# radiocosmology/driftscan

Hardware: AMD Instinct MI355X
Metric: m-blocks/sec (BT-gen + SVD + KL) (higher is better)
Workload: dtype f64

## Files before the change

driftscan_amd/csrc/dm_chol.hip:

```cpp
#include "dm_common.h"
#include "dm_kernels.h"

#include <algorithm>

namespace {

constexpr int NB = 32;

struct chol_desc {
  cplx* A; int ld; int n;
};

__global__ __launch_bounds__(256) void potf2_kernel(const chol_desc* __restrict__ ds, int k0, int* __restrict__ info) {
  __shared__ cplx T[NB][NB + 1];
  __shared__ cplx Lo[NB][NB + 1];
  const chol_desc d = ds[blockIdx.x];
  if (k0 >= d.n) return;
  if (info[blockIdx.x] != 0) return;
  const int nb = min(NB, d.n - k0);
  const int tid = threadIdx.x;
  for (int idx = tid; idx < NB * NB; idx += 256) {
    int r = idx / NB, c = idx % NB;
    T[r][c] = (r < nb && c < nb && c <= r) ? d.A[(size_t)(k0 + r) * d.ld + k0 + c] : make_double2(0.0, 0.0);
    Lo[r][c] = make_double2(0.0, 0.0);
  }
  int fail = 0;
  for (int j = 0; j < nb; ++j) {
    __syncthreads();
    const double djj = T[j][j].x;
    if (!(djj > 0.0) || !isfinite(djj)) {
      fail = j + 1;
      break;
    }
    const double inv = 1.0 / djj, invs = 1.0 / sqrt(djj);
    if (tid >= j && tid < nb) Lo[tid][j] = tid == j ? make_double2(sqrt(djj), 0.0) : cscale(T[tid][j], invs);
    for (int idx = tid; idx < NB * NB; idx += 256) {
      int r = idx / NB, c = idx % NB;
      if (c > j && c <= r && r < nb) T[r][c] = csub(T[r][c], cscale(cmulc(T[r][j], T[c][j]), inv));
    }
  }
  if (fail) {
    if (tid == 0) info[blockIdx.x] = k0 + fail;
    return;
  }
  __syncthreads();
  for (int idx = tid; idx < NB * NB; idx += 256) {
    int r = idx / NB, c = idx % NB;
    if (r < nb && c < nb) {
      cplx v = (c <= r) ? Lo[r][c] : make_double2(0.0, 0.0);
      if (c == r) v.y = 0.0;
      d.A[(size_t)(k0 + r) * d.ld + k0 + c] = v;
    }
  }
}

__global__ __launch_bounds__(256) void panel_trsm_kernel(const chol_desc* __restrict__ ds, int k0,
                                                         const int* __restrict__ info) {
  __shared__ cplx Lk[NB][NB + 1];
  __shared__ cplx R[64][NB + 1];
  const chol_desc d = ds[blockIdx.y];
  if (k0 + NB >= d.n) return;
  if (info[blockIdx.y] != 0) return;
  const int r0 = k0 + NB + blockIdx.x * 64;
  if (r0 >= d.n) return;
  const int tid = threadIdx.x;
  for (int idx = tid; idx < NB * NB; idx += 256) {
    int r = idx / NB, c = idx % NB;
    Lk[r][c] = d.A[(size_t)(k0 + r) * d.ld + k0 + c];
  }
  for (int idx = tid; idx < 64 * NB; idx += 256) {
    int r = idx / NB, c = idx % NB;
    R[r][c] = (r0 + r < d.n) ? d.A[(size_t)(r0 + r) * d.ld + k0 + c] : make_double2(0.0, 0.0);
  }
  __syncthreads();
  if (tid < 64) {
    const int r = tid;
    cplx x[NB];
#pragma unroll
    for (int c = 0; c < NB; ++c) x[c] = R[r][c];
#pragma unroll
    for (int c = 0; c < NB; ++c) {
      x[c] = cscale(x[c], 1.0 / Lk[c][c].x);
#pragma unroll
      for (int j = c + 1; j < NB; ++j) x[j] = csub(x[j], cmulc(x[c], Lk[j][c]));
    }
#pragma unroll
    for (int c = 0; c < NB; ++c) R[r][c] = x[c];
  }
  __syncthreads();
  for (int idx = tid; idx < 64 * NB; idx += 256) {
    int r = idx / NB, c = idx % NB;
    if (r0 + r < d.n) d.A[(size_t)(r0 + r) * d.ld + k0 + c] = R[r][c];
  }
}

__global__ void zero_upper_kernel(const chol_desc* __restrict__ ds) {
  const chol_desc d = ds[blockIdx.z];
  const int r = blockIdx.y, c = blockIdx.x * blockDim.x + threadIdx.x;
  if (r < d.n && c < d.n && c > r) d.A[(size_t)r * d.ld + c] = make_double2(0.0, 0.0);
}

struct trsm_desc {
  const cplx* L; int ldl; int n; cplx* B; int ldb; int nrhs;
};

template <bool CONJTRANS>
__global__ __launch_bounds__(256) void diag_solve_kernel(const trsm_desc* __restrict__ ds, int s, int nblk, int upper_only) {
  __shared__ cplx Lk[NB][NB + 1];
  const trsm_desc d = ds[blockIdx.y];
  int k0;
  if (!CONJTRANS) {
    k0 = s * NB;
  } else {
    const int pn = (d.n + NB - 1) / NB;
    if (s < nblk - pn) return;
    k0 = (pn - 1 - (s - (nblk - pn))) * NB;
  }
  if (k0 >= d.n || k0 < 0) return;
  const int nb = min(NB, d.n - k0);
  const int col = blockIdx.x * 256 + threadIdx.x;
  const int first_col = upper_only ? (k0 / (2 * NB)) * (2 * NB) : 0;
  if ((int)(blockIdx.x + 1) * 256 <= first_col) return;
  for (int idx = threadIdx.x; idx < NB * NB; idx += 256) {
    int r = idx / NB, c = idx % NB;
    Lk[r][c] = (r < nb && c < nb) ? d.L[(size_t)(k0 + r) * d.ldl + k0 + c] : make_double2(0.0, 0.0);
  }
  __syncthreads();
  if (col >= d.nrhs || (col / 64 + 1) * 64 <= first_col) return;
  cplx x[NB];
#pragma unroll
  for (int r = 0; r < NB; ++r) x[r] = (r < nb) ? d.B[(size_t)(k0 + r) * d.ldb + col] : make_double2(0.0, 0.0);
  if (!CONJTRANS) {
#pragma unroll
    for (int r = 0; r < NB; ++r) {
      if (r < nb) {
        x[r] = cscale(x[r], 1.0 / Lk[r][r].x);
#pragma unroll
        for (int j = r + 1; j < NB; ++j) x[j] = csub(x[j], cmul(Lk[j][r], x[r]));
      }
    }
  } else {
#pragma unroll
    for (int rr = 0; rr < NB; ++rr) {
      const int r = NB - 1 - rr;
      if (r < nb) {
        x[r] = cscale(x[r], 1.0 / Lk[r][r].x);
#pragma unroll
        for (int j = 0; j < r; ++j) x[j] = csub(x[j], cmul(cconj(Lk[r][j]), x[r]));
      }
    }
  }
#pragma unroll
  for (int r = 0; r < NB; ++r)
    if (r < nb) d.B[(size_t)(k0 + r) * d.ldb + col] = x[r];
}

}

int dm_potrf_batched(dm_ctx* ctx, const std::vector<dm_mat>& mats, int* info_dev) {
  const int nbatch = (int)mats.size();
  if (nbatch == 0) return DM_OK;
  dm_ws_scope ws_scope__(ctx);
  const size_t mark = ws_scope__.mark;
  std::vector<chol_desc> ds(nbatch);
  int maxn = 0;
  for (int i = 0; i < nbatch; ++i) {
    ds[i] = chol_desc{mats[i].p, mats[i].ld, mats[i].n};
    maxn = std::max(maxn, mats[i].n);
  }
  chol_desc* dd = dm_ws_upload(ctx, ds);
  if (!dd) return DM_ENOMEM;
  DM_HIP(ctx, hipMemsetAsync(info_dev, 0, sizeof(int) * nbatch, ctx->stream));
  dm_gemm_chain chain(ctx);
  for (int pass = 0; pass < 2; ++pass) {
    if (pass == 1) DM_TRY(chain.upload());
    for (int k0 = 0; k0 < maxn; k0 += 2 * NB) {
      for (int half = 0; half < 2; ++half) {
        const int kk = k0 + half * NB;
        if (kk >= maxn) break;
        if (!chain.dry) DM_PLAUNCH(ctx, DM_PROF_CHOL, potf2_kernel, dim3(nbatch), dim3(256), 0, ctx->stream, dd, kk, info_dev);
        if (kk + NB >= maxn) break;
        const int rt = (maxn - kk - NB + 63) / 64;
        if (!chain.dry) DM_PLAUNCH(ctx, DM_PROF_CHOL, panel_trsm_kernel, dim3(rt, nbatch), dim3(256), 0, ctx->stream, dd, kk, info_dev);
        if (half == 0) {
          DM_TRY(chain.gemm([&](std::vector<dm_gemm_desc>& g) {
            for (int i = 0; i < nbatch; ++i) {
              const int rem = mats[i].n - kk - NB;
              if (rem <= 0) continue;
              cplx* L21 = mats[i].p + (size_t)(kk + NB) * mats[i].ld + kk;
              cplx* A22 = mats[i].p + (size_t)(kk + NB) * mats[i].ld + (kk + NB);
              g.push_back(dm_gemm_make(L21, mats[i].ld, 1, false, L21, 1, mats[i].ld, true, A22, mats[i].ld, rem,
                                       std::min(NB, rem), NB, -1.0, 1.0));
            }
          }));
        }
      }
      const int k2 = k0 + 2 * NB;
      if (k2 < maxn) {
        DM_TRY(chain.gemm([&](std::vector<dm_gemm_desc>& g) {
          for (int i = 0; i < nbatch; ++i) {
            const int rem = mats[i].n - k2;
            if (rem <= 0) continue;
            cplx* L21 = mats[i].p + (size_t)k2 * mats[i].ld + k0;
            cplx* A22 = mats[i].p + (size_t)k2 * mats[i].ld + k2;
            g.push_back(dm_gemm_make(L21, mats[i].ld, 1, false, L21, 1, mats[i].ld, true, A22, mats[i].ld, rem, rem,
                                     2 * NB, -1.0, 1.0, nullptr, DM_GEMM_LOWER));
          }
        }));
      }
    }
  }
  DM_PLAUNCH(ctx, DM_PROF_CHOL, zero_upper_kernel, dim3((maxn + 255) / 256, maxn, nbatch), dim3(256), 0, ctx->stream, dd);
  DM_HIP(ctx, hipGetLastError());
  (void)mark;
  return DM_OK;
}

namespace {
int trsm_pass(dm_ctx* ctx, const std::vector<dm_trsm_problem>& probs, bool conjtrans, bool upper_only, dm_gemm_chain& chain,
              const trsm_desc* dd) {
  const int nbatch = (int)probs.size();
  int maxn = 0, maxrhs = 0;
  for (int i = 0; i < nbatch; ++i) {
    maxn = std::max(maxn, probs[i].n);
    maxrhs = std::max(maxrhs, probs[i].nrhs);
  }
  const int ct = (maxrhs + 255) / 256;
  const int NB2 = 2 * NB;
  const int nblk = (maxn + NB2 - 1) / NB2;
  const int nblk32 = (maxn + NB - 1) / NB;
  for (int s = 0; s < nblk; ++s) {
    DM_TRY(chain.gemm([&](std::vector<dm_gemm_desc>& g) {
    for (int i = 0; i < nbatch; ++i) {
      const dm_trsm_problem& P = probs[i];
      const int pn = (P.n + NB2 - 1) / NB2;
      if (!conjtrans) {
        if (s == 0 || s >= pn) continue;
        const int size = s & -s;
        const int r0 = s * NB2, r1 = std::min((s + size) * NB2, P.n);
        const int c0 = (s - size) * NB2;
        const int j0 = upper_only ? std::min(r0, P.nrhs) : 0;
        if (P.nrhs - j0 <= 0) continue;
        g.push_back(dm_gemm_make(P.L + (size_t)r0 * P.ldl + c0, P.ldl, 1, false, P.B + (size_t)c0 * P.ldb + j0, P.ldb, 1,
                                 false, P.B + (size_t)r0 * P.ldb + j0, P.ldb, r1 - r0, P.nrhs - j0, size * NB2, -1.0,
                                 1.0));
      } else {
        if (s < nblk - pn) continue;
        const int u = s - (nblk - pn);
        if (u == 0) continue;
        const int kb = pn - 1 - u;
        const int size = u & -u;
        const int t0 = std::max(kb - size + 1, 0) * NB2, t1 = (kb + 1) * NB2;
        const int k1 = t1, k2 = std::min((kb + 1 + size) * NB2, P.n);
        g.push_back(dm_gemm_make(P.L + (size_t)k1 * P.ldl + t0, 1, P.ldl, true, P.B + (size_t)k1 * P.ldb, P.ldb, 1,
                                 false, P.B + (size_t)t0 * P.ldb, P.ldb, t1 - t0, P.nrhs, k2 - k1, -1.0, 1.0));
      }
    }
    }));
    for (int half = 0; half < 2; ++half) {
      const int h = conjtrans ? 1 - half : half;
      int s32;
      if (!conjtrans) s32 = 2 * s + h;
      else s32 = 2 * s + half;
      if (chain.dry) {
      } else if (!conjtrans)
        DM_PLAUNCH(ctx, DM_PROF_CHOL, diag_solve_kernel<false>, dim3(ct, nbatch), dim3(256), 0, ctx->stream, dd, s32, nblk32,
                           upper_only ? 1 : 0);
      else
        DM_PLAUNCH(ctx, DM_PROF_CHOL, diag_solve_kernel<true>, dim3(ct, nbatch), dim3(256), 0, ctx->stream, dd, s32, 2 * nblk, 0);
      if (half == 0) {
        DM_TRY(chain.gemm([&](std::vector<dm_gemm_desc>& g2) {
        for (int i = 0; i < nbatch; ++i) {
          const dm_trsm_problem& P = probs[i];
          const int pn = (P.n + NB2 - 1) / NB2;
          if (!conjtrans) {
            const int k0 = s * NB2, k1 = k0 + NB;
            if (k1 >= P.n) continue;
            const int nb = std::min(NB, P.n - k1);
            const int j0 = upper_only ? std::min(k0, P.nrhs) : 0;
            if (P.nrhs - j0 <= 0) continue;
            g2.push_back(dm_gemm_make(P.L + (size_t)k1 * P.ldl + k0, P.ldl, 1, false, P.B + (size_t)k0 * P.ldb + j0,
                                      P.ldb, 1, false, P.B + (size_t)k1 * P.ldb + j0, P.ldb, nb, P.nrhs - j0, NB, -1.0,
                                      1.0));
          } else {
            if (s < nblk - pn) continue;
            const int kb = pn - 1 - (s - (nblk - pn));
            const int k0 = kb * NB2, k1 = k0 + NB;
            if (k1 >= P.n) continue;
            const int nb2 = std::min(NB, P.n - k1);
            g2.push_back(dm_gemm_make(P.L + (size_t)k1 * P.ldl + k0, 1, P.ldl, true, P.B + (size_t)k1 * P.ldb, P.ldb,
                                      1, false, P.B + (size_t)k0 * P.ldb, P.ldb, NB, P.nrhs, nb2, -1.0, 1.0));
          }
        }
        }));
      }
    }
  }
  return DM_OK;
}
}

int dm_trsm_plan_build(dm_ctx* ctx, const std::vector<dm_trsm_problem>& probs, bool conjtrans, bool upper_only, dm_trsm_plan& plan) {
  if (conjtrans) upper_only = false;
  plan.probs = probs;
  plan.conjtrans = conjtrans;
  plan.upper_only = upper_only;
  plan.chain.reset(new dm_gemm_chain(ctx));
  plan.empty = true;
  for (const auto& P : probs)
    if (P.n > 0 && P.nrhs > 0) plan.empty = false;
  if (plan.empty) return DM_OK;
  return trsm_pass(ctx, plan.probs, conjtrans, upper_only, *plan.chain, nullptr);
}

int dm_trsm_plan_run(dm_ctx* ctx, dm_trsm_plan& plan) {
  if (plan.empty || !plan.chain) return DM_OK;
  const int nbatch = (int)plan.probs.size();
  std::vector<trsm_desc> ds(nbatch);
  for (int i = 0; i < nbatch; ++i)
    ds[i] = trsm_desc{plan.probs[i].L, plan.probs[i].ldl, plan.probs[i].n, plan.probs[i].B, plan.probs[i].ldb, plan.probs[i].nrhs};
  trsm_desc* dd = dm_ws_upload(ctx, ds);
  if (!dd) return DM_ENOMEM;
  DM_TRY(plan.chain->upload());
  DM_TRY(trsm_pass(ctx, plan.probs, plan.conjtrans, plan.upper_only, *plan.chain, dd));
  DM_HIP(ctx, hipGetLastError());
  return DM_OK;
}

int dm_trsm_left_lower_batched(dm_ctx* ctx, const std::vector<dm_trsm_problem>& probs, bool conjtrans, bool upper_only) {
  dm_trsm_plan plan;
  DM_TRY(dm_trsm_plan_build(ctx, probs, conjtrans, upper_only, plan));
  return dm_trsm_plan_run(ctx, plan);
}
```

Baseline: 1116.

## Use 64-wide diagonal blocks with quad-thread solves in Cholesky and TRSM

Replaces the 32-wide potf2/panel-trsm/diag-solve kernels with 64-wide versions. The diagonal block is stored in packed-triangular shared memory, and each row or column is solved by four cooperating lanes that exchange values with shuffles. This removes the intermediate 32-wide GEMM updates and halves the number of kernel launches per block step. In exchange each diagonal step does more serial work, and the per-thread register arrays and the triangular-index arithmetic add cost.

```diff
diff --git a/driftscan_amd/csrc/dm_chol.hip b/driftscan_amd/csrc/dm_chol.hip
--- a/driftscan_amd/csrc/dm_chol.hip
+++ b/driftscan_amd/csrc/dm_chol.hip
@@ -5,38 +5,39 @@
 
 namespace {
 
-constexpr int NB = 32;
+constexpr int NB2 = 64;
+
+constexpr int TRI64 = NB2 * (NB2 + 1) / 2;
+__device__ __forceinline__ int tri(int r, int c) { return r * (r + 1) / 2 + c; }
 
 struct chol_desc {
   cplx* A; int ld; int n;
 };
 
-__global__ __launch_bounds__(256) void potf2_kernel(const chol_desc* __restrict__ ds, int k0, int* __restrict__ info) {
-  __shared__ cplx T[NB][NB + 1];
-  __shared__ cplx Lo[NB][NB + 1];
+__global__ __launch_bounds__(256) void potf2_64_kernel(const chol_desc* __restrict__ ds, int k0, int* __restrict__ info) {
+  __shared__ cplx T[TRI64];
   const chol_desc d = ds[blockIdx.x];
   if (k0 >= d.n) return;
   if (info[blockIdx.x] != 0) return;
-  const int nb = min(NB, d.n - k0);
+  const int nb = min(NB2, d.n - k0);
   const int tid = threadIdx.x;
-  for (int idx = tid; idx < NB * NB; idx += 256) {
-    int r = idx / NB, c = idx % NB;
-    T[r][c] = (r < nb && c < nb && c <= r) ? d.A[(size_t)(k0 + r) * d.ld + k0 + c] : make_double2(0.0, 0.0);
-    Lo[r][c] = make_double2(0.0, 0.0);
-  }
+  for (int idx = tid; idx < NB2 * NB2; idx += 256) {
+    const int r = idx / NB2, c = idx % NB2;
+    if (c <= r) T[tri(r, c)] = (r < nb) ? d.A[(size_t)(k0 + r) * d.ld + k0 + c] : make_double2(0.0, 0.0);
+  }
+  const int r = tid >> 2, q = tid & 3;
   int fail = 0;
   for (int j = 0; j < nb; ++j) {
     __syncthreads();
-    const double djj = T[j][j].x;
+    const double djj = T[tri(j, j)].x;
     if (!(djj > 0.0) || !isfinite(djj)) {
       fail = j + 1;
       break;
     }
-    const double inv = 1.0 / djj, invs = 1.0 / sqrt(djj);
-    if (tid >= j && tid < nb) Lo[tid][j] = tid == j ? make_double2(sqrt(djj), 0.0) : cscale(T[tid][j], invs);
-    for (int idx = tid; idx < NB * NB; idx += 256) {
-      int r = idx / NB, c = idx % NB;
-      if (c > j && c <= r && r < nb) T[r][c] = csub(T[r][c], cscale(cmulc(T[r][j], T[c][j]), inv));
+    const double inv = 1.0 / djj;
+    if (r > j && r < nb) {
+      const cplx trj = T[tri(r, j)];
+      for (int c = j + 1 + q; c <= r; c += 4) T[tri(r, c)] = csub(T[tri(r, c)], cscale(cmulc(trj, T[tri(c, j)]), inv));
     }
   }
   if (fail) {
@@ -44,54 +45,77 @@
     return;
   }
   __syncthreads();
-  for (int idx = tid; idx < NB * NB; idx += 256) {
-    int r = idx / NB, c = idx % NB;
-    if (r < nb && c < nb) {
-      cplx v = (c <= r) ? Lo[r][c] : make_double2(0.0, 0.0);
-      if (c == r) v.y = 0.0;
-      d.A[(size_t)(k0 + r) * d.ld + k0 + c] = v;
-    }
-  }
-}
-
-__global__ __launch_bounds__(256) void panel_trsm_kernel(const chol_desc* __restrict__ ds, int k0,
-                                                         const int* __restrict__ info) {
-  __shared__ cplx Lk[NB][NB + 1];
-  __shared__ cplx R[64][NB + 1];
+  for (int idx = tid; idx < NB2 * NB2; idx += 256) {
+    const int rr = idx / NB2, c = idx % NB2;
+    if (rr < nb && c < nb) {
+      cplx v = make_double2(0.0, 0.0);
+      if (c == rr) v.x = sqrt(T[tri(c, c)].x);
+      else if (c < rr) v = cscale(T[tri(rr, c)], 1.0 / sqrt(T[tri(c, c)].x));
+      d.A[(size_t)(k0 + rr) * d.ld + k0 + c] = v;
+    }
+  }
+}
+
+template <bool BACK, bool CONJL>
+__device__ __forceinline__ void quad_solve64(const cplx* Lk, const double* rdiag, int nb, int q, cplx (&x)[NB2 / 4]) {
+  constexpr int NQ = NB2 / 4;
+#pragma unroll
+  for (int rr = 0; rr < NB2; ++rr) {
+    const int r = BACK ? NB2 - 1 - rr : rr;
+    if (r < nb) {
+      const int ir = r / 4;
+      const cplx v = cscale(x[ir], rdiag[r]);
+      cplx xr;
+      xr.x = __shfl(v.x, r & 3, 4);
+      xr.y = __shfl(v.y, r & 3, 4);
+      if (q == (r & 3)) x[ir] = xr;
+      if (!BACK) {
+#pragma unroll
+        for (int i = ir; i < NQ; ++i) {
+          const int j = 4 * i + q;
+          if (i > ir || q > (r & 3)) {
+            const cplx l = Lk[tri(j, r)];
+            x[i] = csub(x[i], cmul(CONJL ? cconj(l) : l, xr));
+          }
+        }
+      } else {
+#pragma unroll
+        for (int i = 0; i <= ir; ++i) {
+          const int j = 4 * i + q;
+          if (i < ir || q < (r & 3)) x[i] = csub(x[i], cmul(cconj(Lk[tri(r, j)]), xr));
+        }
+      }
+    }
+  }
+}
+
+__global__ __launch_bounds__(256) void panel_trsm64_kernel(const chol_desc* __restrict__ ds, int k0,
+                                                           const int* __restrict__ info) {
+  __shared__ cplx Lk[TRI64];
   const chol_desc d = ds[blockIdx.y];
-  if (k0 + NB >= d.n) return;
+  if (k0 + NB2 >= d.n) return;
   if (info[blockIdx.y] != 0) return;
-  const int r0 = k0 + NB + blockIdx.x * 64;
+  const int r0 = k0 + NB2 + blockIdx.x * 64;
   if (r0 >= d.n) return;
   const int tid = threadIdx.x;
-  for (int idx = tid; idx < NB * NB; idx += 256) {
-    int r = idx / NB, c = idx % NB;
-    Lk[r][c] = d.A[(size_t)(k0 + r) * d.ld + k0 + c];
-  }
-  for (int idx = tid; idx < 64 * NB; idx += 256) {
-    int r = idx / NB, c = idx % NB;
-    R[r][c] = (r0 + r < d.n) ? d.A[(size_t)(r0 + r) * d.ld + k0 + c] : make_double2(0.0, 0.0);
-  }
+  for (int idx = tid; idx < NB2 * NB2; idx += 256) {
+    const int r = idx / NB2, c = idx % NB2;
+    if (c <= r) Lk[tri(r, c)] = d.A[(size_t)(k0 + r) * d.ld + k0 + c];
+  }
+  __shared__ double rdiag[NB2];
+  if (tid < NB2) rdiag[tid] = 1.0 / d.A[(size_t)(k0 + tid) * d.ld + k0 + tid].x;
   __syncthreads();
-  if (tid < 64) {
-    const int r = tid;
-    cplx x[NB];
-#pragma unroll
-    for (int c = 0; c < NB; ++c) x[c] = R[r][c];
-#pragma unroll
-    for (int c = 0; c < NB; ++c) {
-      x[c] = cscale(x[c], 1.0 / Lk[c][c].x);
-#pragma unroll
-      for (int j = c + 1; j < NB; ++j) x[j] = csub(x[j], cmulc(x[c], Lk[j][c]));
-    }
-#pragma unroll
-    for (int c = 0; c < NB; ++c) R[r][c] = x[c];
-  }
-  __syncthreads();
-  for (int idx = tid; idx < 64 * NB; idx += 256) {
-    int r = idx / NB, c = idx % NB;
-    if (r0 + r < d.n) d.A[(size_t)(r0 + r) * d.ld + k0 + c] = R[r][c];
-  }
+  const int row = r0 + (tid >> 2), q = tid & 3;
+  if (row >= d.n) return;
+  cplx* a = d.A + (size_t)row * d.ld + k0;
+  cplx x[NB2 / 4];
+#pragma unroll
+  for (int i = 0; i < NB2 / 4; ++i) x[i] = a[4 * i + q];
+  int nb = NB2;
+  asm volatile("" : "+s"(nb));
+  quad_solve64<false, true>(Lk, rdiag, nb, q, x);
+#pragma unroll
+  for (int i = 0; i < NB2 / 4; ++i) a[4 * i + q] = x[i];
 }
 
 __global__ void zero_upper_kernel(const chol_desc* __restrict__ ds) {
@@ -105,54 +129,39 @@
 };
 
 template <bool CONJTRANS>
-__global__ __launch_bounds__(256) void diag_solve_kernel(const trsm_desc* __restrict__ ds, int s, int nblk, int upper_only) {
-  __shared__ cplx Lk[NB][NB + 1];
+__global__ __launch_bounds__(256) void diag_solve64_kernel(const trsm_desc* __restrict__ ds, int s, int nblk, int upper_only) {
+  __shared__ cplx Lk[TRI64];
   const trsm_desc d = ds[blockIdx.y];
   int k0;
   if (!CONJTRANS) {
-    k0 = s * NB;
+    k0 = s * NB2;
   } else {
-    const int pn = (d.n + NB - 1) / NB;
+    const int pn = (d.n + NB2 - 1) / NB2;
     if (s < nblk - pn) return;
-    k0 = (pn - 1 - (s - (nblk - pn))) * NB;
+    k0 = (pn - 1 - (s - (nblk - pn))) * NB2;
   }
   if (k0 >= d.n || k0 < 0) return;
-  const int nb = min(NB, d.n - k0);
-  const int col = blockIdx.x * 256 + threadIdx.x;
-  const int first_col = upper_only ? (k0 / (2 * NB)) * (2 * NB) : 0;
-  if ((int)(blockIdx.x + 1) * 256 <= first_col) return;
-  for (int idx = threadIdx.x; idx < NB * NB; idx += 256) {
-    int r = idx / NB, c = idx % NB;
-    Lk[r][c] = (r < nb && c < nb) ? d.L[(size_t)(k0 + r) * d.ldl + k0 + c] : make_double2(0.0, 0.0);
-  }
+  const int nb = min(NB2, d.n - k0);
+  const int col = blockIdx.x * 64 + (threadIdx.x >> 2), q = threadIdx.x & 3;
+  const int first_col = upper_only ? k0 : 0;
+  if ((int)(blockIdx.x + 1) * 64 <= first_col) return;
+  for (int idx = threadIdx.x; idx < NB2 * NB2; idx += 256) {
+    const int r = idx / NB2, c = idx % NB2;
+    if (c <= r) Lk[tri(r, c)] = (r < nb) ? d.L[(size_t)(k0 + r) * d.ldl + k0 + c] : make_double2(0.0, 0.0);
+  }
+  __shared__ double rdiag[NB2];
+  if (threadIdx.x < nb) rdiag[threadIdx.x] = 1.0 / d.L[(size_t)(k0 + threadIdx.x) * d.ldl + k0 + threadIdx.x].x;
   __syncthreads();
-  if (col >= d.nrhs || (col / 64 + 1) * 64 <= first_col) return;
-  cplx x[NB];
-#pragma unroll
-  for (int r = 0; r < NB; ++r) x[r] = (r < nb) ? d.B[(size_t)(k0 + r) * d.ldb + col] : make_double2(0.0, 0.0);
-  if (!CONJTRANS) {
-#pragma unroll
-    for (int r = 0; r < NB; ++r) {
-      if (r < nb) {
-        x[r] = cscale(x[r], 1.0 / Lk[r][r].x);
-#pragma unroll
-        for (int j = r + 1; j < NB; ++j) x[j] = csub(x[j], cmul(Lk[j][r], x[r]));
-      }
-    }
-  } else {
-#pragma unroll
-    for (int rr = 0; rr < NB; ++rr) {
-      const int r = NB - 1 - rr;
-      if (r < nb) {
-        x[r] = cscale(x[r], 1.0 / Lk[r][r].x);
-#pragma unroll
-        for (int j = 0; j < r; ++j) x[j] = csub(x[j], cmul(cconj(Lk[r][j]), x[r]));
-      }
-    }
-  }
-#pragma unroll
-  for (int r = 0; r < NB; ++r)
-    if (r < nb) d.B[(size_t)(k0 + r) * d.ldb + col] = x[r];
+  if (col >= d.nrhs || col < first_col) return;
+  cplx* b = d.B + (size_t)k0 * d.ldb + col;
+  const size_t ldb = d.ldb;
+  cplx x[NB2 / 4];
+#pragma unroll
+  for (int i = 0; i < NB2 / 4; ++i) x[i] = (4 * i + q < nb) ? b[(4 * i + q) * ldb] : make_double2(0.0, 0.0);
+  quad_solve64<CONJTRANS, false>(Lk, rdiag, nb, q, x);
+#pragma unroll
+  for (int i = 0; i < NB2 / 4; ++i)
+    if (4 * i + q < nb) b[(4 * i + q) * ldb] = x[i];
 }
 
 }
@@ -174,40 +183,22 @@
   dm_gemm_chain chain(ctx);
   for (int pass = 0; pass < 2; ++pass) {
     if (pass == 1) DM_TRY(chain.upload());
-    for (int k0 = 0; k0 < maxn; k0 += 2 * NB) {
-      for (int half = 0; half < 2; ++half) {
-        const int kk = k0 + half * NB;
-        if (kk >= maxn) break;
-        if (!chain.dry) DM_PLAUNCH(ctx, DM_PROF_CHOL, potf2_kernel, dim3(nbatch), dim3(256), 0, ctx->stream, dd, kk, info_dev);
-        if (kk + NB >= maxn) break;
-        const int rt = (maxn - kk - NB + 63) / 64;
-        if (!chain.dry) DM_PLAUNCH(ctx, DM_PROF_CHOL, panel_trsm_kernel, dim3(rt, nbatch), dim3(256), 0, ctx->stream, dd, kk, info_dev);
-        if (half == 0) {
-          DM_TRY(chain.gemm([&](std::vector<dm_gemm_desc>& g) {
-            for (int i = 0; i < nbatch; ++i) {
-              const int rem = mats[i].n - kk - NB;
-              if (rem <= 0) continue;
-              cplx* L21 = mats[i].p + (size_t)(kk + NB) * mats[i].ld + kk;
-              cplx* A22 = mats[i].p + (size_t)(kk + NB) * mats[i].ld + (kk + NB);
-              g.push_back(dm_gemm_make(L21, mats[i].ld, 1, false, L21, 1, mats[i].ld, true, A22, mats[i].ld, rem,
-                                       std::min(NB, rem), NB, -1.0, 1.0));
-            }
-          }));
+    for (int k0 = 0; k0 < maxn; k0 += NB2) {
+      if (!chain.dry) DM_PLAUNCH(ctx, DM_PROF_CHOL, potf2_64_kernel, dim3(nbatch), dim3(256), 0, ctx->stream, dd, k0, info_dev);
+      const int k2 = k0 + NB2;
+      if (k2 >= maxn) break;
+      const int rt = (maxn - k2 + 63) / 64;
+      if (!chain.dry) DM_PLAUNCH(ctx, DM_PROF_CHOL, panel_trsm64_kernel, dim3(rt, nbatch), dim3(256), 0, ctx->stream, dd, k0, info_dev);
+      DM_TRY(chain.gemm([&](std::vector<dm_gemm_desc>& g) {
+        for (int i = 0; i < nbatch; ++i) {
+          const int rem = mats[i].n - k2;
+          if (rem <= 0) continue;
+          cplx* L21 = mats[i].p + (size_t)k2 * mats[i].ld + k0;
+          cplx* A22 = mats[i].p + (size_t)k2 * mats[i].ld + k2;
+          g.push_back(dm_gemm_make(L21, mats[i].ld, 1, false, L21, 1, mats[i].ld, true, A22, mats[i].ld, rem, rem, NB2, -1.0,
+                                   1.0, nullptr, DM_GEMM_LOWER));
         }
-      }
-      const int k2 = k0 + 2 * NB;
-      if (k2 < maxn) {
-        DM_TRY(chain.gemm([&](std::vector<dm_gemm_desc>& g) {
-          for (int i = 0; i < nbatch; ++i) {
-            const int rem = mats[i].n - k2;
-            if (rem <= 0) continue;
-            cplx* L21 = mats[i].p + (size_t)k2 * mats[i].ld + k0;
-            cplx* A22 = mats[i].p + (size_t)k2 * mats[i].ld + k2;
-            g.push_back(dm_gemm_make(L21, mats[i].ld, 1, false, L21, 1, mats[i].ld, true, A22, mats[i].ld, rem, rem,
-                                     2 * NB, -1.0, 1.0, nullptr, DM_GEMM_LOWER));
-          }
-        }));
-      }
+      }));
     }
   }
   DM_PLAUNCH(ctx, DM_PROF_CHOL, zero_upper_kernel, dim3((maxn + 255) / 256, maxn, nbatch), dim3(256), 0, ctx->stream, dd);
@@ -225,10 +216,8 @@
     maxn = std::max(maxn, probs[i].n);
     maxrhs = std::max(maxrhs, probs[i].nrhs);
   }
-  const int ct = (maxrhs + 255) / 256;
-  const int NB2 = 2 * NB;
+  const int ct = (maxrhs + 63) / 64;
   const int nblk = (maxn + NB2 - 1) / NB2;
-  const int nblk32 = (maxn + NB - 1) / NB;
   for (int s = 0; s < nblk; ++s) {
     DM_TRY(chain.gemm([&](std::vector<dm_gemm_desc>& g) {
     for (int i = 0; i < nbatch; ++i) {
@@ -257,44 +246,12 @@
       }
     }
     }));
-    for (int half = 0; half < 2; ++half) {
-      const int h = conjtrans ? 1 - half : half;
-      int s32;
-      if (!conjtrans) s32 = 2 * s + h;
-      else s32 = 2 * s + half;
-      if (chain.dry) {
-      } else if (!conjtrans)
-        DM_PLAUNCH(ctx, DM_PROF_CHOL, diag_solve_kernel<false>, dim3(ct, nbatch), dim3(256), 0, ctx->stream, dd, s32, nblk32,
-                           upper_only ? 1 : 0);
-      else
-        DM_PLAUNCH(ctx, DM_PROF_CHOL, diag_solve_kernel<true>, dim3(ct, nbatch), dim3(256), 0, ctx->stream, dd, s32, 2 * nblk, 0);
-      if (half == 0) {
-        DM_TRY(chain.gemm([&](std::vector<dm_gemm_desc>& g2) {
-        for (int i = 0; i < nbatch; ++i) {
-          const dm_trsm_problem& P = probs[i];
-          const int pn = (P.n + NB2 - 1) / NB2;
-          if (!conjtrans) {
-            const int k0 = s * NB2, k1 = k0 + NB;
-            if (k1 >= P.n) continue;
-            const int nb = std::min(NB, P.n - k1);
-            const int j0 = upper_only ? std::min(k0, P.nrhs) : 0;
-            if (P.nrhs - j0 <= 0) continue;
-            g2.push_back(dm_gemm_make(P.L + (size_t)k1 * P.ldl + k0, P.ldl, 1, false, P.B + (size_t)k0 * P.ldb + j0,
-                                      P.ldb, 1, false, P.B + (size_t)k1 * P.ldb + j0, P.ldb, nb, P.nrhs - j0, NB, -1.0,
-                                      1.0));
-          } else {
-            if (s < nblk - pn) continue;
-            const int kb = pn - 1 - (s - (nblk - pn));
-            const int k0 = kb * NB2, k1 = k0 + NB;
-            if (k1 >= P.n) continue;
-            const int nb2 = std::min(NB, P.n - k1);
-            g2.push_back(dm_gemm_make(P.L + (size_t)k1 * P.ldl + k0, 1, P.ldl, true, P.B + (size_t)k1 * P.ldb, P.ldb,
-                                      1, false, P.B + (size_t)k0 * P.ldb, P.ldb, NB, P.nrhs, nb2, -1.0, 1.0));
-          }
-        }
-        }));
-      }
-    }
+    if (chain.dry) {
+    } else if (!conjtrans)
+      DM_PLAUNCH(ctx, DM_PROF_CHOL, diag_solve64_kernel<false>, dim3(ct, nbatch), dim3(256), 0, ctx->stream, dd, s, nblk,
+                 upper_only ? 1 : 0);
+    else
+      DM_PLAUNCH(ctx, DM_PROF_CHOL, diag_solve64_kernel<true>, dim3(ct, nbatch), dim3(256), 0, ctx->stream, dd, s, nblk, 0);
   }
   return DM_OK;
 }
```

Result: no change. 1135 (median of 6 runs) (+1.7%).
